# shanglianlm0525/CvPytorch

Hardware: AMD Instinct MI355X
Metric: images/sec/node train step, YOLOv5-s@640 (value: batch resident in HBM when the timed region starts; with_h2d.value: the same step fed from pinned host memory inside the region) & DeepLabv3+R50@1024x512 (config3_deeplabv3plus_r50.value) (higher is better)
Workload: dtype bf16; 1 GPU; coco_yolov5_s.yml YOLOv5-s 640x640 bf16 train step (fwd+loss+bwd+SGD-nesterov+EMA), per-GPU batch 64, synthetic COCO-shape tensors resident in HBM; global_batch=64, parallelism=dp1, launch=hipGraph replay of the whole step, world=1, transport=none (single process), grad_buckets=0, sync_bn=False, deterministic=True

## Files before the change

### cvpytorch_amd/csrc/api.hip

```cpp
#include <string.h>

#include <string>

#include "common.h"
#include "conv_plan.h"

namespace cvhip {

static thread_local std::string g_last_error = "";

void set_last_error(const char* what, hipError_t e) {
  g_last_error = std::string(what) + ": " + hipGetErrorString(e);
}

int check_launch(const char* what) {
  hipError_t e = hipGetLastError();
  if (e != hipSuccess) {
    set_last_error(what, e);
    return CVHIP_ERR_LAUNCH;
  }
  return CVHIP_OK;
}

__global__ __launch_bounds__(256) void zero_fill_kernel(uint32_t* p, size_t n_words, int tail_half) {
// ... 433 lines not shown
  p.res_ld = addend_ld;
  p.y_vec_ok = ((d->x_ld & 3) == 0) && ((((uintptr_t)dx) & 7) == 0);
  return launch_igemm(p, (hipStream_t)stream);
}

int cvhip_conv2d_dgrad(const cvhip_conv_desc* d, const void* dy, const void* w_dgrad, void* dx, void* stream) {
  return dgrad_impl(d, dy, w_dgrad, nullptr, 0, dx, stream);
}

int cvhip_conv2d_dgrad_add(const cvhip_conv_desc* d, const void* dy, const void* w_dgrad, const void* addend, int32_t addend_ld, void* dx,
                           void* stream) {
  if (!addend) return CVHIP_ERR_INVALID;
  return dgrad_impl(d, dy, w_dgrad, addend, addend_ld, dx, stream);
}

int cvhip_conv2d_wgrad(const cvhip_conv_desc* d, const void* x, const void* dy, float* dw, int accumulate, void* stream) {
  int st = validate_dense_desc(d);
  if (st) return st;
  if (!x || !dy || !dw) return CVHIP_ERR_INVALID;
  if ((d->K & 7) || (d->y_ld & 7)) return CVHIP_ERR_UNSUPPORTED;
  if ((((uintptr_t)x) & 15) || (((uintptr_t)dy) & 15)) return CVHIP_ERR_INVALID;
  hipStream_t s = (hipStream_t)stream;
  if (!accumulate) {
    int zs = zero_fill(dw, sizeof(float) * (size_t)d->K * d->R * d->S * d->C, s);
    if (zs) return zs;
  }
  return launch_wgrad(d, x, dy, dw, s);
}

int64_t cvhip_conv2d_wgrad_det_workspace_bytes(const cvhip_conv_desc* d) {
// ... 37 lines not shown
```

### cvpytorch_amd/csrc/conv1x1_stream.hip

```cpp
#include <stdlib.h>

#include "common.h"
#include "conv_plan.h"

namespace cvhip {

constexpr int kS1MaxLds = 72 * 1024;
constexpr int kS1MaxBlocks = 512;
constexpr int kS1MinTiles = 192;


template <int NV>
__device__ __forceinline__ void s1_act_vec(float (&v)[NV], int act, float ap) {
  switch (act) {
    case CVHIP_ACT_NONE: break;
    case CVHIP_ACT_RELU:
#pragma unroll
      for (int q = 0; q < NV; ++q) v[q] = act_fwd(v[q], CVHIP_ACT_RELU, ap);
      break;
    case CVHIP_ACT_SILU:
#pragma unroll
      for (int q = 0; q < NV; ++q) v[q] = act_fwd(v[q], CVHIP_ACT_SILU, ap);
      break;
    case CVHIP_ACT_LEAKY:
// ... 267 lines not shown
          u1 += red[(w * BN + t) * 2 + 0];
          u2 += red[(w * BN + t) * 2 + 1];
        }
        if (p.stats_acc) {
          acc_add2(reinterpret_cast<double*>(p.stats), blockIdx.x, p.stats_ld, n0 + t, u1, u2);
        } else {
          float* dst = p.stats + (int64_t)blockIdx.x * 2 * p.Nout;
          dst[n0 + t] = u1;
          dst[p.Nout + n0 + t] = u2;
        }
      }
    }
  }
}


static int s1x1_mode() {
  static int v = -1;
  if (v < 0) {
    const char* e = getenv("CVHIP_S1X1");
    v = e ? atoi(e) : 1;
  }
  return v;
}

static int s1x1_nf(int Nout, int Cin, bool stats) {
  if (Nout <= 32) return 2;
  if (Nout <= 64) return 4;
  if (Nout > 128 && Nout <= 256 && !stats && 256 * (((Cin + 31) & ~31) * 2 + 16) <= kS1MaxLds) return 16;
  return 8;
// ... 17 lines not shown

static bool s1x1_structural(const IgemmParams& p) {
  if (p.ncls != 1) return false;
  const IgemmClass& c = p.cls[0];
  return c.TR == 1 && c.TS == 1 && p.in_sh == 1 && p.in_sw == 1 && p.out_sh == 1 && p.out_sw == 1 && c.dh0 == 0 && c.dw0 == 0 &&
         c.out_oh == 0 && c.out_ow == 0 && c.OHi == p.OH && c.OWi == p.OW && p.IH == p.OH && p.IW == p.OW && (p.x_ld & 7) == 0;
}

static int s1x1_lds(int bn, int cin_pad, bool pro) {
  int lds = bn * (cin_pad * 2 + 16) + 5 * bn * (int)sizeof(float) + (pro ? 2 * cin_pad * (int)sizeof(float) : 0);
  if (lds < 4 * bn * 2 * (int)sizeof(float)) lds = 4 * bn * 2 * (int)sizeof(float);
  return lds;
}
constexpr int kS1MaxLdsPro = kS1MaxLds + 4096;

template <int NF, int STATS, bool EPI = false, bool PRO = false>
static int launch_s1(const IgemmParams& p, int blocks, int ntiles, hipStream_t stream) {
  constexpr int MF = 2;
  const int bn = NF * 16;
  const int cin_pad = (p.Cin + 31) & ~31;
  const int lds = s1x1_lds(bn, cin_pad, PRO);
  if (lds > kS1MaxLdsPro) return CVHIP_ERR_UNSUPPORTED;
  auto kern = conv1x1_stream_kernel<NF, MF, STATS, EPI, PRO>;
  static bool attr_done[64] = {};
  int devid = 0;
  (void)hipGetDevice(&devid);
  bool& attr_set = attr_done[devid & 63];
  if (!attr_set) {
    hipError_t e = hipFuncSetAttribute(reinterpret_cast<const void*>(kern), hipFuncAttributeMaxDynamicSharedMemorySize, kS1MaxLds + 4096);
    if (e != hipSuccess) {
      set_last_error("hipFuncSetAttribute(conv1x1_stream_kernel)", e);
      return CVHIP_ERR_LAUNCH;
    }
    attr_set = true;
  }
  const int vec16 = ((p.y_ld & 7) == 0) && ((((uintptr_t)p.y) & 15) == 0);
  const IgemmKernArgs k = narrow_plan(p, 0, 1);
  hipLaunchKernelGGL(kern, dim3(blocks, cdiv(p.Nout, bn)), dim3(256), lds, stream, k, ntiles, vec16);
  return check_launch("conv1x1_stream_kernel");
}

bool stream1x1_prologue_ok(const IgemmParams& p, bool stats) {
  if (!s1x1_structural(p)) return false;
  if (stream1x1_blocks(p.Nout, p.Cin, p.cls[0].M, stats) <= 0) return false;
  const int nf = s1x1_nf(p.Nout, p.Cin, stats);
  if (nf == 16) return false;
  return s1x1_lds(nf * 16, (p.Cin + 31) & ~31, true) <= kS1MaxLdsPro;
}

int try_launch_stream1x1(const IgemmParams& p, hipStream_t stream) {
  if (!s1x1_structural(p)) return -1;
  const int64_t M = p.cls[0].M;
  const int blocks = stream1x1_blocks(p.Nout, p.Cin, M, p.stats != nullptr);
  if (blocks <= 0) return -1;
// ... 38 lines not shown
```

### cvpytorch_amd/csrc/conv_plan.h

```cpp
#pragma once
#include <hip/hip_runtime.h>
#include <stdint.h>

#include "common.h"

namespace cvhip {

constexpr int kMaxClasses = 16;

struct IgemmClass {
  int TR, TS;
  int dh0, dh_step;
  int dw0, dw_step;
  int out_oh, out_ow;
  int OHi, OWi;
  int M;
  int tile_begin;
  int64_t w_off;
  unsigned ts_magic;
  unsigned ohw_mul, ohw_sh, ow_mul, ow_sh;
  int r0, r_step, s0, s_step;
};

struct IgemmCommon {
// ... 129 lines not shown
    return 0;
  }
  *r0 = first;
  *d0 = (ph + pad - first * dil) / stride;
  return (R - 1 - first) / step + 1;
}

int validate_dense_desc(const cvhip_conv_desc* d);
void plan_fprop(const cvhip_conv_desc* d, IgemmParams* p);
int plan_dgrad(const cvhip_conv_desc* d, IgemmParams* p);
int igemm_block_m(int Nout, int64_t M, int Ktot);
int launch_igemm(IgemmParams& p, hipStream_t stream);
int stream1x1_blocks(int Nout, int Cin, int64_t M, bool stats);
int try_launch_stream1x1(const IgemmParams& p, hipStream_t stream);
bool stream1x1_prologue_ok(const IgemmParams& p, bool stats);
int stem_blocks(int C, int x_ld, int K, int R, int S, int sh, int sw, int dh, int dw, int N, int OH, int OW);
int try_launch_stem(const IgemmParams& p, hipStream_t stream);
struct StemWgradBn {
  const void* y;
  int y_ld;
  const float *scale, *shift, *mean, *invstd;
  const double* acc;
  int acc_ld;
  int act;
  float act_param;
  float *dgamma_out, *dbeta_out;
  int accumulate;
};
int try_launch_stem_wgrad(const cvhip_conv_desc* d, const void* x, const void* dy, float* dw, hipStream_t stream, const float* x_image = nullptr,
                          int x_planes = 0, const StemWgradBn* bn = nullptr);
// ... 8 lines not shown
```

### cvpytorch_amd/csrc/f16_names.h

```cpp
#pragma once
#define cvhip_adamw_ema cvhip_adamw_ema_f16
#define cvhip_add2d cvhip_add2d_f16
#define cvhip_add_act_fwd cvhip_add_act_fwd_f16
#define cvhip_bn_acc_shards cvhip_bn_acc_shards_f16
#define cvhip_bn_act_bwd_apply cvhip_bn_act_bwd_apply_f16
#define cvhip_bn_act_bwd_apply_acc cvhip_bn_act_bwd_apply_acc_f16
#define cvhip_bn_act_bwd_partial cvhip_bn_act_bwd_partial_f16
#define cvhip_bn_act_bwd_sums_acc cvhip_bn_act_bwd_sums_acc_f16
#define cvhip_bn_act_fwd cvhip_bn_act_fwd_f16
#define cvhip_bn_act_fwd_acc cvhip_bn_act_fwd_acc_f16
#define cvhip_bn_act_fwd_acc_lazyres cvhip_bn_act_fwd_acc_lazyres_f16
#define cvhip_bn_add_act_fwd cvhip_bn_add_act_fwd_f16
#define cvhip_bn_bwd_finalize cvhip_bn_bwd_finalize_f16
#define cvhip_bn_eval_scale_shift cvhip_bn_eval_scale_shift_f16
#define cvhip_bn_finalize cvhip_bn_finalize_f16
#define cvhip_bn_finalize_acc cvhip_bn_finalize_acc_f16
#define cvhip_bn_stats_partial cvhip_bn_stats_partial_f16
#define cvhip_bn_tail_bwd_sums_acc cvhip_bn_tail_bwd_sums_acc_f16
#define cvhip_box_iou cvhip_box_iou_f16
#define cvhip_channel_scale_bwd_ds cvhip_channel_scale_bwd_ds_f16
#define cvhip_colreduce_rows cvhip_colreduce_rows_f16
#define cvhip_colsum_finalize cvhip_colsum_finalize_f16
#define cvhip_colsum_partial cvhip_colsum_partial_f16
#define cvhip_conv1x1_bwd_fused cvhip_conv1x1_bwd_fused_f16
#define cvhip_conv1x1_bwd_fused_acc cvhip_conv1x1_bwd_fused_acc_f16
#define cvhip_conv1x1_bwd_fused_lazy cvhip_conv1x1_bwd_fused_lazy_f16
#define cvhip_conv1x1_bwd_fused_ok cvhip_conv1x1_bwd_fused_ok_f16
#define cvhip_conv1x1_bwd_fused_split cvhip_conv1x1_bwd_fused_split_f16
#define cvhip_conv1x1_stream_blocks cvhip_conv1x1_stream_blocks_f16
#define cvhip_conv1x1_stream_prologue_ok cvhip_conv1x1_stream_prologue_ok_f16
#define cvhip_conv2d_band_plan cvhip_conv2d_band_plan_f16
#define cvhip_conv2d_dgrad cvhip_conv2d_dgrad_f16
#define cvhip_conv2d_dgrad_add cvhip_conv2d_dgrad_add_f16
#define cvhip_conv2d_dgrad_plan cvhip_conv2d_dgrad_plan_f16
#define cvhip_conv2d_dgrad_weight_elems cvhip_conv2d_dgrad_weight_elems_f16
#define cvhip_conv2d_fprop cvhip_conv2d_fprop_f16
#define cvhip_conv2d_fprop_acc cvhip_conv2d_fprop_acc_f16
#define cvhip_conv2d_fprop_fused cvhip_conv2d_fprop_fused_f16
#define cvhip_conv2d_fprop_prologue_ok cvhip_conv2d_fprop_prologue_ok_f16
#define cvhip_conv2d_fprop_stats_rows cvhip_conv2d_fprop_stats_rows_f16
#define cvhip_conv2d_out_hw cvhip_conv2d_out_hw_f16
#define cvhip_conv2d_patch_plan cvhip_conv2d_patch_plan_f16
#define cvhip_conv2d_prep_weights cvhip_conv2d_prep_weights_f16
// ... 78 lines not shown
```

### cvpytorch_amd/lib.py

```python
import ctypes as C
import os

import torch

_HERE = os.path.dirname(os.path.abspath(__file__))
LIB_PATH = os.environ.get("CVHIP_LIB") or os.path.join(_HERE, "libcvhip.so")

OK, ERR_INVALID, ERR_UNSUPPORTED, ERR_LAUNCH = 0, -1, -2, -3
ACT_NONE, ACT_RELU, ACT_SILU, ACT_LEAKY, ACT_SIGMOID, ACT_HSWISH = 0, 1, 2, 3, 4, 5
DTYPE_F32, DTYPE_F64, DTYPE_I32, DTYPE_BF16, DTYPE_U8 = 0, 1, 2, 3, 4
RED_SUM, RED_MAX, RED_MIN = 0, 1, 2
DGRAD_CLASS_INTS = 12
REDUCE_SCRATCH_ROWS = 64
YOLO_BIAS_ROWS = 256
BN_ACC_SHARDS = 16


class CvhipError(RuntimeError):
    pass


class ConvDesc(C.Structure):
    _fields_ = [(n, C.c_int32) for n in (
        "N", "C", "H", "W", "K", "R", "S", "stride_h", "stride_w", "pad_h", "pad_w", "dil_h", "dil_w",
# ... 60 lines not shown
    "cvhip_conv2d_dgrad_plan": (_i32, [_dp, C.POINTER(_i32), _i32]),
    "cvhip_div31_consts": (_i32, [_i32, C.POINTER(C.c_uint32), C.POINTER(C.c_uint32)]),
    "cvhip_conv2d_prep_weights": (_i32, [_dp, _p, _p, _p, _p]),
    "cvhip_prep_plan_item_bytes": (_i32, []),
    "cvhip_prep_plan_build": (_i32, [_p, _i32, _p, C.POINTER(_i32)]),
    "cvhip_prep_plan_run": (_i32, [_p, _i32, _i32, _p]),
    "cvhip_conv2d_fprop": (_i32, [_dp, _p, _p, _p, _p, _p, _p]),
    "cvhip_conv2d_fprop_fused": (_i32, [_dp, _p, _p, _p, C.POINTER(ConvFuse), _p]),
    "cvhip_conv2d_wgrad_image": (_i32, [_dp, _p, _i32, _p, _p, _p]),
    "cvhip_conv2d_fprop_prologue_ok": (_i32, [_dp, _i32]),
    "cvhip_conv2d_patch_plan": (_i32, [_dp, _i32, C.POINTER(_i32), _i32]),
    "cvhip_conv2d_band_plan": (_i32, [_dp, _i32, C.POINTER(_i32)]),
    "cvhip_conv2d_wgrad_band_plan": (_i32, [_dp, C.POINTER(_i32)]),
    "cvhip_conv1x1_stream_prologue_ok": (_i32, [_dp, _i32]),
    "cvhip_conv2d_wgrad_stem_bn": (_i32, [_dp, _p, _p, _i32, _p, _p, _p, _p, _p, _p, _p, _i32, _p, _p, _i32, _i32, _f32, _p, _p]),
    "cvhip_bn_finalize_acc": (_i32, [_p, _i32, _i32, _i64, _p, _p, _p, _p, _f32, _f32, _p, _p, _p, _p, _p]),
    "cvhip_bn_act_fwd_acc_lazyres": (_i32, [_p, _i32, _p, _i32, _i64, _i32, _p, _i32, _i64, _p, _p, _p, _p, _f32, _f32, _p, _p, _p, _p, _i32, _f32,
                                     _p, _i32, _p, _p, _p]),
    "cvhip_conv1x1_bwd_fused_split": (_i32, [_dp, _p, _i32, _p, _i32, _i32, _p, _p, _i32, _p, _p, _p, _p, _p, _p, _p, _i32, _p, _p, _i32, _i32, _f32, _p,
                                      _i32, _p, _i32, _p, C.POINTER(LazyIn), _p]),
    "cvhip_conv1x1_bwd_fused_lazy": (_i32, [_dp, _p, _i32, _p, _i32, _i32, _p, _p, _p, _p, _p, _p, _p, _p, _i32, _p, _p, _i32, _i32, _f32, _p, _i32,
                                     _p, _i32, _p, C.POINTER(LazyIn), _p]),
    "cvhip_conv2d_dgrad": (_i32, [_dp, _p, _p, _p, _p]),
    "cvhip_conv2d_dgrad_add": (_i32, [_dp, _p, _p, _p, _i32, _p, _p]),
    "cvhip_conv2d_wgrad": (_i32, [_dp, _p, _p, _p, _i32, _p]),
    "cvhip_conv2d_wgrad_det_workspace_bytes": (_i64, [_dp]),
    "cvhip_conv2d_wgrad_det": (_i32, [_dp, _p, _p, _p, _i32, _p, _i64, _p]),
    "cvhip_conv1x1_bwd_fused_ok": (_i32, [_dp]),
    "cvhip_conv1x1_bwd_fused": (_i32, [_dp, _p, _i32, _p, _i32, _i32, _p, _p, _p, _p, _p, _p, _p, _p, _p, _i32, _f32, _p, _i32, _p, _i32,
                                _p, _p]),
# ... 211 lines not shown
```

### cvpytorch_amd/ops.py

```python
import ctypes as C

import torch

from . import lib as L

ACT_DTYPE = torch.bfloat16
_weights_epoch = 0
_stats_epoch = [0]


def set_precision(p):
    global ACT_DTYPE
    L.set_precision(p)
    ACT_DTYPE = torch.float16 if p == "fp16" else torch.bfloat16
    bump_weights_epoch()
    _desc_cache.clear()


def precision():
    return L.PRECISION


def bump_weights_epoch():
    global _weights_epoch
# ... 684 lines not shown
                    g_out.data_ptr(), b_out.data_ptr(), int(accum), act, act_param, tmp.data_ptr(), st,
                    nbytes=2.0 * (N * H * W * Cc + 2 * N * P * Q * K))
    except L.CvhipError as e:
        if "unsupported" not in str(e):
            raise
        return False
    arena = cfg.arena
    direct_w = arena is not None and cfg.gw is not None and tuple(cfg.gw.shape) == tuple(weight.shape)
    if direct_w:
        L.call("cvhip_f32_unpad_add", tmp.data_ptr(), cfg.gw.data_ptr(), K, R * S, Cc, Cg, st)
        _mark(arena, cfg.idx_w)
        return None
    dw = zero_fill(torch.empty((K, Cg, R, S), dtype=torch.float32, device=dev, memory_format=torch.channels_last))
    L.call("cvhip_f32_unpad_add", tmp.data_ptr(), dw.data_ptr(), K, R * S, Cc, Cg, st)
    return dw if dw.dtype == weight.dtype else dw.to(weight.dtype)


def _bwd1x1_ok(ctx, cfg, x, need_dx, need_dw, need_db, segs):
    N, Cc, H, W, K, R, S, P, Q, Kp, x_ld, Cg = ctx.geom
    if _DETERMINISTIC:
        return False
    if ctx.depthwise or R != 1 or S != 1 or Kp != K or Cg != Cc or ctx.c_orig != Cc or not (need_dx and need_dw):
        return False
    if (ctx.has_bias and need_db) or ctx.w_dgrad is None or x.data_ptr() % 16 or x_ld % 8:
        return False
    for d, d_ld in segs:
        if d_ld % 8 or d.data_ptr() % 16:
            return False
    desc = conv_desc(N, Cc, H, W, K, R, S, cfg.stride, cfg.pad, cfg.dil, 1, x_ld, Kp)
    return bool(L.load().cvhip_conv1x1_bwd_fused_ok(C.byref(desc)))
# ... 480 lines not shown
                    need_dg = need_dbeta = False
                    for i in cfg.idx_bn:
                        arena.mark_ready(i)
                ag, ab = (dgamma, dbeta) if cfg.sync is None else _sync_bwd_sums(dgamma, dbeta, cfg.sync)
            dx, dw = _bwd1x1(ctx, cfg, x, y, weight, ((dz, dz_ld),), K, stats, ctx.train_bn, ag, ab, act, act_param)
            dres = dz if ctx.has_res else None
            if dres is not None and cfg.res_link is not None and cfg.res_link.ok:
                cfg.res_link.g = dres
                dres = None
            return dx, dw, None, (dgamma if need_dg else None), (dbeta if need_dbeta else None), None, None, dres, None
        if pointwise:
            if Kp != K:
                dy = zero_fill(torch.empty((N, P, Q, Kp), dtype=ACT_DTYPE, device=dev)).permute(0, 3, 1, 2)[:, :K]
            else:
                dy = empty_nhwc(N, K, P, Q, dev)
            if acc_b is not None:
                _timed_ew("bn_act_bwd_apply(ew_kernel<1>)", 6.0 * M * K, "cvhip_bn_act_bwd_apply_acc", dz.data_ptr(), dz_ld, y.data_ptr(), Kp, dy.data_ptr(), Kp, M, K,
                          stats[2].data_ptr(), stats[3].data_ptr(), stats[0].data_ptr(), stats[1].data_ptr(), acc_b.data_ptr(), K,
                          g_out.data_ptr(), b_out.data_ptr(), accum, act, act_param, st)
                if direct_bn:
                    need_dg = need_dbeta = False
                    for i in cfg.idx_bn:
                        arena.mark_ready(i)
            elif ctx.train_bn:
                rows = _colreduce_rows(M, K)
                partial = torch.empty((rows + L.REDUCE_SCRATCH_ROWS, 2, K), dtype=torch.float32, device=dev)
                _timed_ew("bn_act_bwd_sums(colreduce_kernel<1>)", 4.0 * M * K, "cvhip_bn_act_bwd_partial", dz.data_ptr(), dz_ld, y.data_ptr(), Kp, M, K, stats[2].data_ptr(),
                       stats[3].data_ptr(), stats[0].data_ptr(), stats[1].data_ptr(), act, act_param,
                       partial.data_ptr(), st)
                dgamma = torch.empty((K,), dtype=torch.float32, device=dev)
                dbeta = torch.empty((K,), dtype=torch.float32, device=dev)
                L.call("cvhip_bn_bwd_finalize", partial.data_ptr(), rows, K, dgamma.data_ptr(), dbeta.data_ptr(),
                       cfg.gg.data_ptr() if direct_bn else None, cfg.gbeta.data_ptr() if direct_bn else None, st)
                if direct_bn:
                    need_dg = need_dbeta = False
                    for i in cfg.idx_bn:
                        arena.mark_ready(i)
                ag, ab = (dgamma, dbeta) if cfg.sync is None else _sync_bwd_sums(dgamma, dbeta, cfg.sync)
                _timed_ew("bn_act_bwd_apply(ew_kernel<1>)", 6.0 * M * K, "cvhip_bn_act_bwd_apply", dz.data_ptr(), dz_ld, y.data_ptr(), Kp, dy.data_ptr(), Kp, M, K,
                          stats[2].data_ptr(), stats[3].data_ptr(), stats[0].data_ptr(), stats[1].data_ptr(),
                       ag.data_ptr(), ab.data_ptr(), act, act_param, st)
            else:
                sc = stats[2].data_ptr() if stats is not None else None
                sh = stats[3].data_ptr() if stats is not None else None
                L.call("cvhip_bn_act_bwd_apply", dz.data_ptr(), dz_ld, y.data_ptr(), Kp, dy.data_ptr(), Kp, M, K, sc, sh,
                       None, None, None, None, act, act_param, st)
            dy_ld = Kp
        else:
            dy, dy_ld = dz, dz_ld
            if dy_ld % 8 != 0 or dy.data_ptr() % 16 != 0 or (Kp != K and dy_ld < Kp):
                buf = zero_fill(torch.empty((N, P, Q, Kp), dtype=ACT_DTYPE, device=dev))
                L.call("cvhip_copy2d", dy.data_ptr(), dy_ld, buf.data_ptr(), Kp, M, K, st)
                dy, dy_ld = buf.permute(0, 3, 1, 2)[:, :K], Kp
        dx, dw, dbias = _conv_grads(ctx, x, weight, dy, dy_ld, need_dx, need_dw, need_db)
        dres = dz if ctx.has_res else None
        if dres is not None and cfg.res_link is not None and cfg.res_link.ok:
            cfg.res_link.g = dres
            dres = None
        if dx is not None and ctx.c_orig != Cc:
            dx = dx[:, :ctx.c_orig]
        return dx, dw, dbias, (dgamma if need_dg else None), (dbeta if need_dbeta else None), None, None, dres, None


def _lazy_consumer_ok(x, K, R, S, has_bias, cfg, lz):
    if not _LAZY or _DETERMINISTIC or not torch.is_grad_enabled() or not x.requires_grad:
        return False
    if cfg.groups != 1 or (R, S) != (1, 1) or tuple(cfg.stride) != (1, 1) or tuple(cfg.pad) != (0, 0) or has_bias:
        return False
    if not (cfg.has_bn and cfg.bn_training) or cfg.sync is not None or not _BN_ACC or K > 128 or K % 8:
# ... 1192 lines not shown
```

### include/cvhip.h

```cpp
#if !defined(CVHIP_H_) || defined(CVHIP_REDECLARE_F16)
#ifndef CVHIP_H_
#define CVHIP_H_
#endif

#include <stddef.h>
#include <stdint.h>

#ifdef __cplusplus
extern "C" {
#endif

#define CVHIP_VERSION 100

#define CVHIP_OK 0
#define CVHIP_ERR_INVALID (-1)
#define CVHIP_ERR_UNSUPPORTED (-2)
#define CVHIP_ERR_LAUNCH (-3)

#define CVHIP_ACT_NONE 0
#define CVHIP_ACT_RELU 1
#define CVHIP_ACT_SILU 2
#define CVHIP_ACT_LEAKY 3
#define CVHIP_ACT_SIGMOID 4
#define CVHIP_ACT_HSWISH 5
// ... 377 lines not shown
  const float* scale;
  const float* shift;
  int32_t act;
  float act_param;
  int32_t c_lo;
  int32_t c_hi;
} cvhip_lazy_in;
#endif
int cvhip_conv2d_fprop_fused(const cvhip_conv_desc* d, const void* x, const void* w, void* y, const cvhip_conv_fuse* f, void* stream);
int cvhip_conv2d_wgrad_image(const cvhip_conv_desc* d, const float* x_nchw, int32_t planes, const void* dy, float* dw, void* stream);
int cvhip_conv2d_wgrad_stem_bn(const cvhip_conv_desc* d, const void* x, const float* x_nchw, int32_t planes, const void* dz, const void* y,
                               const float* scale, const float* shift, const float* mean, const float* invstd, const double* acc, int32_t acc_ld,
                               float* dgamma_out, float* dbeta_out, int32_t accumulate, int32_t act, float act_param, float* dw, void* stream);
int cvhip_conv2d_fprop_prologue_ok(const cvhip_conv_desc* d, int with_z_out);
int cvhip_conv1x1_stream_prologue_ok(const cvhip_conv_desc* d, int with_stats);
int cvhip_bn_finalize_acc(const double* acc, int32_t acc_ld, int32_t C, int64_t count, const float* gamma, const float* beta,
                          float* running_mean, float* running_var, float momentum, float eps, float* mean, float* invstd, float* scale,
                          float* shift, void* stream);
int cvhip_bn_act_fwd_acc_lazyres(const void* y, int32_t ld_y, void* z, int32_t ld_z, int64_t M, int32_t C, const double* acc, int32_t acc_ld,
                                 int64_t count, const float* gamma, const float* beta, float* running_mean, float* running_var,
                                 float momentum, float eps, float* mean, float* invstd, float* scale, float* shift, int32_t act,
                                 float act_param, const void* residual_raw, int32_t ld_res, const float* res_scale, const float* res_shift,
                                 void* stream);
int cvhip_conv1x1_bwd_fused_split(const cvhip_conv_desc* d, const void* dz0, int32_t dz0_ld, const void* dz1, int32_t dz1_ld, int32_t k_split,
                                  const void* y, const void* y1, int32_t y1_ld, const void* x, const void* w_dgrad, const float* scale,
                                  const float* shift, const float* mean, const float* invstd, const double* acc, int32_t acc_ld,
                                  float* dgamma_out, float* dbeta_out, int32_t accumulate, int32_t act, float act_param, const void* addend,
                                  int32_t addend_ld, void* dx, int32_t dx_ld, float* dw, const cvhip_lazy_in* xin, void* stream);
int cvhip_conv1x1_bwd_fused_lazy(const cvhip_conv_desc* d, const void* dz0, int32_t dz0_ld, const void* dz1, int32_t dz1_ld, int32_t k_split,
                                 const void* y, const void* x_raw, const void* w_dgrad, const float* scale, const float* shift, const float* mean,
// ... 18 lines not shown
```

### include/cvhip_f16.h

```cpp
#ifndef CVHIP_F16_H_
#define CVHIP_F16_H_
#include "cvhip.h"
#define cvhip_adamw_ema cvhip_adamw_ema_f16
#define cvhip_add2d cvhip_add2d_f16
#define cvhip_add_act_fwd cvhip_add_act_fwd_f16
#define cvhip_bn_acc_shards cvhip_bn_acc_shards_f16
#define cvhip_bn_act_bwd_apply cvhip_bn_act_bwd_apply_f16
#define cvhip_bn_act_bwd_apply_acc cvhip_bn_act_bwd_apply_acc_f16
#define cvhip_bn_act_bwd_partial cvhip_bn_act_bwd_partial_f16
#define cvhip_bn_act_bwd_sums_acc cvhip_bn_act_bwd_sums_acc_f16
#define cvhip_bn_act_fwd cvhip_bn_act_fwd_f16
#define cvhip_bn_act_fwd_acc cvhip_bn_act_fwd_acc_f16
#define cvhip_bn_act_fwd_acc_lazyres cvhip_bn_act_fwd_acc_lazyres_f16
#define cvhip_bn_add_act_fwd cvhip_bn_add_act_fwd_f16
#define cvhip_bn_bwd_finalize cvhip_bn_bwd_finalize_f16
#define cvhip_bn_eval_scale_shift cvhip_bn_eval_scale_shift_f16
#define cvhip_bn_finalize cvhip_bn_finalize_f16
#define cvhip_bn_finalize_acc cvhip_bn_finalize_acc_f16
#define cvhip_bn_stats_partial cvhip_bn_stats_partial_f16
#define cvhip_bn_tail_bwd_sums_acc cvhip_bn_tail_bwd_sums_acc_f16
#define cvhip_box_iou cvhip_box_iou_f16
#define cvhip_channel_scale_bwd_ds cvhip_channel_scale_bwd_ds_f16
#define cvhip_colreduce_rows cvhip_colreduce_rows_f16
#define cvhip_colsum_finalize cvhip_colsum_finalize_f16
#define cvhip_colsum_partial cvhip_colsum_partial_f16
#define cvhip_conv1x1_bwd_fused cvhip_conv1x1_bwd_fused_f16
#define cvhip_conv1x1_bwd_fused_acc cvhip_conv1x1_bwd_fused_acc_f16
#define cvhip_conv1x1_bwd_fused_lazy cvhip_conv1x1_bwd_fused_lazy_f16
#define cvhip_conv1x1_bwd_fused_ok cvhip_conv1x1_bwd_fused_ok_f16
#define cvhip_conv1x1_bwd_fused_split cvhip_conv1x1_bwd_fused_split_f16
#define cvhip_conv1x1_stream_blocks cvhip_conv1x1_stream_blocks_f16
#define cvhip_conv1x1_stream_prologue_ok cvhip_conv1x1_stream_prologue_ok_f16
#define cvhip_conv2d_band_plan cvhip_conv2d_band_plan_f16
#define cvhip_conv2d_dgrad cvhip_conv2d_dgrad_f16
#define cvhip_conv2d_dgrad_add cvhip_conv2d_dgrad_add_f16
#define cvhip_conv2d_dgrad_plan cvhip_conv2d_dgrad_plan_f16
#define cvhip_conv2d_dgrad_weight_elems cvhip_conv2d_dgrad_weight_elems_f16
#define cvhip_conv2d_fprop cvhip_conv2d_fprop_f16
#define cvhip_conv2d_fprop_acc cvhip_conv2d_fprop_acc_f16
#define cvhip_conv2d_fprop_fused cvhip_conv2d_fprop_fused_f16
#define cvhip_conv2d_fprop_prologue_ok cvhip_conv2d_fprop_prologue_ok_f16
#define cvhip_conv2d_fprop_stats_rows cvhip_conv2d_fprop_stats_rows_f16
#define cvhip_conv2d_out_hw cvhip_conv2d_out_hw_f16
#define cvhip_conv2d_patch_plan cvhip_conv2d_patch_plan_f16
#define cvhip_conv2d_prep_weights cvhip_conv2d_prep_weights_f16
// ... 93 lines not shown
#undef cvhip_bn_eval_scale_shift
#undef cvhip_bn_finalize
#undef cvhip_bn_finalize_acc
#undef cvhip_bn_stats_partial
#undef cvhip_bn_tail_bwd_sums_acc
#undef cvhip_box_iou
#undef cvhip_channel_scale_bwd_ds
#undef cvhip_colreduce_rows
#undef cvhip_colsum_finalize
#undef cvhip_colsum_partial
#undef cvhip_conv1x1_bwd_fused
#undef cvhip_conv1x1_bwd_fused_acc
#undef cvhip_conv1x1_bwd_fused_lazy
#undef cvhip_conv1x1_bwd_fused_ok
#undef cvhip_conv1x1_bwd_fused_split
#undef cvhip_conv1x1_stream_blocks
#undef cvhip_conv1x1_stream_prologue_ok
#undef cvhip_conv2d_band_plan
#undef cvhip_conv2d_dgrad
#undef cvhip_conv2d_dgrad_add
#undef cvhip_conv2d_dgrad_plan
#undef cvhip_conv2d_dgrad_weight_elems
#undef cvhip_conv2d_fprop
#undef cvhip_conv2d_fprop_acc
#undef cvhip_conv2d_fprop_fused
#undef cvhip_conv2d_fprop_prologue_ok
#undef cvhip_conv2d_fprop_stats_rows
#undef cvhip_conv2d_out_hw
#undef cvhip_conv2d_patch_plan
#undef cvhip_conv2d_prep_weights
// ... 79 lines not shown
```

Before: 5015 images/sec.

## Fuse BN-activation backward apply into the 1x1 conv dgrad stream kernel

Adds a variant of the streaming 1x1 conv kernel that loads dz and y, applies the BN+activation backward transform in registers, writes du (from the first N-block only), and feeds the result straight into the MFMA dgrad GEMM. The Python backward uses it instead of the separate elementwise bn_act_bwd_apply kernel whenever the geometry qualifies. dx then comes from the fused kernel and the regular dgrad is skipped. This saves one kernel launch and the re-read of du by dgrad. The cost is that each N-block recomputes the transform and loads y alongside dz, which adds register pressure and redundant work when Nout spans several blocks.

```diff
diff --git a/cvpytorch_amd/csrc/api.hip b/cvpytorch_amd/csrc/api.hip
--- a/cvpytorch_amd/csrc/api.hip
+++ b/cvpytorch_amd/csrc/api.hip
@@ -471,6 +471,62 @@
   return dgrad_impl(d, dy, w_dgrad, addend, addend_ld, dx, stream);
 }
 
+static bool dgb_unpadded(const cvhip_conv_desc* d) { return (d->k_valid <= 0 || d->k_valid == d->K) && (d->c_valid <= 0 || d->c_valid == d->C); }
+
+int cvhip_conv1x1_dgrad_bnact_ok(const cvhip_conv_desc* d) {
+  if (validate_dense_desc(d) || (d->K & 7) || (d->y_ld & 7) || !dgb_unpadded(d)) return 0;
+  IgemmParams p;
+  plan_dgrad(d, &p);
+  return stream1x1_dgrad_bnact_ok(p) ? 1 : 0;
+}
+
+int cvhip_conv1x1_dgrad_bnact(const cvhip_conv_desc* d, const void* dz, int32_t dz_ld, const void* y, const void* w_dgrad, const float* scale,
+                              const float* shift, const float* mean, const float* invstd, const double* acc, int32_t acc_ld, float* dgamma,
+                              float* dbeta, int32_t accumulate, int32_t act, float act_param, const void* addend, int32_t addend_ld, void* du,
+                              int32_t du_ld, void* dx, void* stream) {
+  int st = validate_dense_desc(d);
+  if (st) return st;
+  if (!dz || !y || !w_dgrad || !du || !dx || !scale || !shift || !mean || !invstd) return CVHIP_ERR_INVALID;
+  if (acc ? (acc_ld < d->K || (((uintptr_t)acc) & 7)) : (!dgamma || !dbeta)) return CVHIP_ERR_INVALID;
+  if ((d->K & 7) || (d->y_ld & 7) || (dz_ld & 7) || (du_ld & 7) || !dgb_unpadded(d)) return CVHIP_ERR_UNSUPPORTED;
+  if (dz_ld < d->K || du_ld < d->K || (addend && addend_ld < d->C)) return CVHIP_ERR_INVALID;
+  if ((((uintptr_t)dz) & 15) || (((uintptr_t)y) & 15) || (((uintptr_t)du) & 15) || (((uintptr_t)w_dgrad) & 15)) return CVHIP_ERR_INVALID;
+  cvhip_conv_desc dd = *d;
+  dd.y_ld = dz_ld;
+  IgemmParams p;
+  plan_dgrad(&dd, &p);
+  p.x = (const h16_t*)dz;
+  p.w = (const h16_t*)w_dgrad;
+  p.y = (h16_t*)dx;
+  p.bias = nullptr;
+  p.stats = nullptr;
+  p.stats_acc = 0;
+  p.stats_ld = d->C;
+  p.res = (const h16_t*)addend;
+  p.res_ld = addend_ld;
+  p.y_vec_ok = ((d->x_ld & 3) == 0) && ((((uintptr_t)dx) & 7) == 0);
+  S1BwdArgs bw{};
+  bw.y = (const h16_t*)y;
+  bw.y_ld = d->y_ld;
+  bw.du = (h16_t*)du;
+  bw.du_ld = du_ld;
+  bw.scale = scale;
+  bw.shift = shift;
+  bw.mean = mean;
+  bw.invstd = invstd;
+  bw.acc = acc;
+  bw.acc_ld = acc_ld;
+  bw.dgamma = acc ? nullptr : dgamma;
+  bw.dbeta = acc ? nullptr : dbeta;
+  bw.dgamma_out = acc ? dgamma : nullptr;
+  bw.dbeta_out = acc ? dbeta : nullptr;
+  bw.accumulate = accumulate;
+  bw.ap = act_param;
+  const int64_t M = (int64_t)p.cls[0].M;
+  bw.inv_count = 1.f / (float)M;
+  return launch_stream1x1_dgrad_bnact(p, bw, act, (hipStream_t)stream);
+}
+
 int cvhip_conv2d_wgrad(const cvhip_conv_desc* d, const void* x, const void* dy, float* dw, int accumulate, void* stream) {
   int st = validate_dense_desc(d);
   if (st) return st;
diff --git a/cvpytorch_amd/csrc/conv1x1_stream.hip b/cvpytorch_amd/csrc/conv1x1_stream.hip
--- a/cvpytorch_amd/csrc/conv1x1_stream.hip
+++ b/cvpytorch_amd/csrc/conv1x1_stream.hip
@@ -305,6 +305,230 @@
   }
 }
 
+template <int ACT>
+struct S1Bwd {
+  static constexpr int act = ACT;
+};
+template <int NF, int MF, typename TAG>
+__global__ __launch_bounds__(256, 2) void conv1x1_stream_kernel(const IgemmKernArgs p, int ntiles, int vec16, const S1BwdArgs bw) {
+  constexpr int BN = NF * 16;
+  constexpr int RT = 64 * MF;
+  constexpr int KC = 128 / MF;
+  constexpr int KS = KC / 32;
+  extern __shared__ __attribute__((aligned(16))) unsigned char smem[];
+
+  const int t = threadIdx.x;
+  const int lane = t & 63;
+  const int wave = __builtin_amdgcn_readfirstlane(t >> 6);
+  const int r = lane & 15, g = lane >> 4;
+  const int Cin = p.Cin;
+  const int M = p.cls[0].M;
+  const int cin_pad = (Cin + 31) & ~31;
+  const int brow = cin_pad * 2 + 16;
+  const int nkc = (cin_pad + KC - 1) / KC;
+  const int n0 = blockIdx.y * BN;
+  const int my_tiles = (ntiles - (int)blockIdx.x + (int)gridDim.x - 1) / (int)gridDim.x;
+  const int total = my_tiles * nkc;
+
+  h16x8 buf0[MF][KS], buf1[MF][KS], ybuf0[MF][KS], ybuf1[MF][KS];
+
+  int ld_tile = blockIdx.x, ld_kc = 0;
+  auto load = [&](h16x8 (&dst)[MF][KS], h16x8 (&ydst)[MF][KS]) {
+    const int row0 = ld_tile * RT + wave * (MF * 16) + r;
+    const int kbase = ld_kc * KC + g * 8;
+#pragma unroll
+    for (int b = 0; b < MF; ++b) {
+      int m = row0 + b * 16;
+      m = m < M ? m : M - 1;
+      const h16_t* src = p.x + (int64_t)m * p.x_ld;
+      const h16_t* ysrc = bw.y + (int64_t)m * bw.y_ld;
+#pragma unroll
+      for (int ks = 0; ks < KS; ++ks) {
+        int kk = kbase + ks * 32;
+        kk = kk < Cin ? kk : 0;
+        dst[b][ks] = *reinterpret_cast<const h16x8*>(src + kk);
+        ydst[b][ks] = *reinterpret_cast<const h16x8*>(ysrc + kk);
+      }
+    }
+    if (++ld_kc == nkc) {
+      ld_kc = 0;
+      ld_tile += gridDim.x;
+    }
+  };
+  load(buf0, ybuf0);
+
+  {
+    const int cpr = cin_pad >> 3;
+    const int nchunks = BN * cpr;
+    constexpr int U = 8;
+    for (int q0 = t; q0 < nchunks; q0 += 256 * U) {
+      uint4 v[U];
+      int dst[U];
+#pragma unroll
+      for (int u = 0; u < U; ++u) {
+        const int q = q0 + u * 256;
+        const int L = q / cpr;
+        const int kq = q - L * cpr;
+        const int a = L >> 4, i = L & 15;
+        const int ch = n0 + (a >> 1) * 32 + (i >> 2) * 8 + (a & 1) * 4 + (i & 3);
+        dst[u] = q < nchunks ? L * brow + kq * 16 : -1;
+        v[u] = make_uint4(0u, 0u, 0u, 0u);
+        if (q < nchunks && ch < p.Nout && kq * 8 < Cin) v[u] = *reinterpret_cast<const uint4*>(p.w + (int64_t)ch * Cin + kq * 8);
+      }
+#pragma unroll
+      for (int u = 0; u < U; ++u)
+        if (dst[u] >= 0) *reinterpret_cast<uint4*>(smem + dst[u]) = v[u];
+    }
+  }
+  float* const scst = reinterpret_cast<float*>(smem + BN * brow);
+  for (int c = t; c < cin_pad; c += 256) {
+    const int cc = c < Cin ? c : Cin - 1;
+    float k1, k2;
+    if (bw.acc) {
+      double s1, s2;
+      acc_fold2(bw.acc, bw.acc_ld, cc, s1, s2);
+      k1 = (float)s1 * bw.inv_count;
+      k2 = (float)s2 * bw.inv_count;
+      if (blockIdx.x == 0 && blockIdx.y == 0 && c < Cin) {
+        if (bw.dbeta_out) bw.dbeta_out[c] = bw.accumulate ? bw.dbeta_out[c] + (float)s1 : (float)s1;
+        if (bw.dgamma_out) bw.dgamma_out[c] = bw.accumulate ? bw.dgamma_out[c] + (float)s2 : (float)s2;
+      }
+    } else {
+      k1 = bw.dbeta[cc] * bw.inv_count;
+      k2 = bw.dgamma[cc] * bw.inv_count;
+    }
+    scst[c] = bw.scale[cc];
+    scst[cin_pad + c] = bw.shift[cc];
+    scst[2 * cin_pad + c] = bw.mean[cc];
+    scst[3 * cin_pad + c] = bw.invstd[cc];
+    scst[4 * cin_pad + c] = k1;
+    scst[5 * cin_pad + c] = k2;
+  }
+  __syncthreads();
+
+  f32x4 acc[NF][MF];
+#pragma unroll
+  for (int a = 0; a < NF; ++a)
+#pragma unroll
+    for (int b = 0; b < MF; ++b) acc[a][b] = f32x4{0.f, 0.f, 0.f, 0.f};
+
+  const unsigned char* const wlane = smem + r * brow + g * 16;
+  int cp_tile = blockIdx.x, cp_kc = 0;
+
+  auto xform = [&](h16x8 (&buf)[MF][KS], const h16x8 (&ybuf)[MF][KS]) {
+    const int kbase = cp_kc * KC + g * 8;
+    const int ksn = min(KS, (cin_pad - cp_kc * KC) >> 5);
+    const int row0 = cp_tile * RT + wave * (MF * 16) + r;
+    const bool keep = blockIdx.y == 0;
+#pragma unroll
+    for (int ks = 0; ks < KS; ++ks) {
+      const int kk = kbase + ks * 32;
+      if (ks < ksn && kk < Cin) {
+        uint32_t dw[MF][4], yw[MF][4];
+#pragma unroll
+        for (int b = 0; b < MF; ++b) {
+          const uint4 d4 = __builtin_bit_cast(uint4, buf[b][ks]), y4 = __builtin_bit_cast(uint4, ybuf[b][ks]);
+          dw[b][0] = d4.x; dw[b][1] = d4.y; dw[b][2] = d4.z; dw[b][3] = d4.w;
+          yw[b][0] = y4.x; yw[b][1] = y4.y; yw[b][2] = y4.z; yw[b][3] = y4.w;
+        }
+#pragma unroll
+        for (int h = 0; h < 2; ++h) {
+          const float* cs = scst + kk + 4 * h;
+          const f32x4 sc = *reinterpret_cast<const f32x4*>(cs), sh = *reinterpret_cast<const f32x4*>(cs + cin_pad);
+          const f32x4 mu = *reinterpret_cast<const f32x4*>(cs + 2 * cin_pad), is = *reinterpret_cast<const f32x4*>(cs + 3 * cin_pad);
+          const f32x4 k1 = *reinterpret_cast<const f32x4*>(cs + 4 * cin_pad), k2 = *reinterpret_cast<const f32x4*>(cs + 5 * cin_pad);
+#pragma unroll
+          for (int b = 0; b < MF; ++b)
+#pragma unroll
+            for (int q = 0; q < 2; ++q) {
+              const int e = 2 * q, w = 2 * h + q;
+              const f32x2 o = bnact_bwd_apply2<TAG::act, true>(unpack_pair(dw[b][w]), unpack_pair(yw[b][w]), f32x2{sc[e], sc[e + 1]},
+                                                               f32x2{sh[e], sh[e + 1]}, f32x2{mu[e], mu[e + 1]}, f32x2{is[e], is[e + 1]},
+                                                               f32x2{k1[e], k1[e + 1]}, f32x2{k2[e], k2[e + 1]}, bw.ap);
+              dw[b][w] = pack2(o.x, o.y);
+            }
+        }
+#pragma unroll
+        for (int b = 0; b < MF; ++b) {
+          const uint4 o4 = make_uint4(dw[b][0], dw[b][1], dw[b][2], dw[b][3]);
+          buf[b][ks] = __builtin_bit_cast(h16x8, o4);
+          const int m = row0 + b * 16;
+          if (keep && m < M) *reinterpret_cast<uint4*>(bw.du + (int64_t)m * bw.du_ld + kk) = o4;
+        }
+      }
+    }
+  };
+
+  auto compute = [&](const h16x8 (&src)[MF][KS]) {
+    const unsigned char* wk = wlane + cp_kc * (KC * 2);
+    const int ksn = min(KS, (cin_pad - cp_kc * KC) >> 5);
+#pragma unroll
+    for (int ks = 0; ks < KS; ++ks) {
+      if (ks < ksn) {
+#pragma unroll
+        for (int a = 0; a < NF; ++a) {
+          const h16x8 wb = *reinterpret_cast<const h16x8*>(wk + a * 16 * brow + ks * 64);
+#pragma unroll
+          for (int b = 0; b < MF; ++b) acc[a][b] = CVHIP_MFMA_16X16X32(wb, src[b][ks], acc[a][b], 0, 0, 0);
+        }
+      }
+    }
+    if (++cp_kc < nkc) return;
+    const int row0 = cp_tile * RT + wave * (MF * 16) + r;
+#pragma unroll
+    for (int b = 0; b < MF; ++b) {
+      const int m = row0 + b * 16;
+      h16_t* yrow = p.y + (int64_t)m * p.y_ld;
+#pragma unroll
+      for (int j = 0; j < NF / 2; ++j) {
+        const int ch0 = n0 + j * 32 + g * 8;
+        f32x8 v;
+#pragma unroll
+        for (int q = 0; q < 4; ++q) {
+          v.v[q] = acc[2 * j][b][q];
+          v.v[4 + q] = acc[2 * j + 1][b][q];
+        }
+        if (p.res && m < M) {
+          const h16_t* rrow = p.res + (int64_t)m * p.res_ld + ch0;
+          if (ch0 + 7 < p.Nout && (p.res_ld & 7) == 0 && ((((uintptr_t)p.res) & 15) == 0)) {
+            const f32x8 rv = unpack8(*reinterpret_cast<const uint4*>(rrow));
+#pragma unroll
+            for (int q = 0; q < 8; ++q) v.v[q] += rv.v[q];
+          } else {
+#pragma unroll
+            for (int q = 0; q < 8; ++q)
+              if (ch0 + q < p.Nout) v.v[q] += (float)rrow[q];
+          }
+        }
+        if (m < M) {
+          if (vec16 && ch0 + 7 < p.Nout) {
+            *reinterpret_cast<uint4*>(yrow + ch0) = pack8(v);
+          } else {
+#pragma unroll
+            for (int q = 0; q < 8; ++q)
+              if (ch0 + q < p.Nout) yrow[ch0 + q] = (h16_t)v.v[q];
+          }
+        }
+      }
+    }
+#pragma unroll
+    for (int a = 0; a < NF; ++a)
+#pragma unroll
+      for (int b = 0; b < MF; ++b) acc[a][b] = f32x4{0.f, 0.f, 0.f, 0.f};
+    cp_kc = 0;
+    cp_tile += gridDim.x;
+  };
+
+  for (int it = 0; it < total; it += 2) {
+    load(buf1, ybuf1);
+    xform(buf0, ybuf0);
+    compute(buf0);
+    load(buf0, ybuf0);
+    xform(buf1, ybuf1);
+    compute(buf1);
+  }
+}
+
 
 static int s1x1_mode() {
   static int v = -1;
@@ -352,6 +576,21 @@
 }
 constexpr int kS1MaxLdsPro = kS1MaxLds + 4096;
 
+static int s1_grant_lds(const void* kern, bool (&done)[64]) {
+  int devid = 0;
+  (void)hipGetDevice(&devid);
+  bool& attr_set = done[devid & 63];
+  if (!attr_set) {
+    hipError_t e = hipFuncSetAttribute(kern, hipFuncAttributeMaxDynamicSharedMemorySize, kS1MaxLdsPro);
+    if (e != hipSuccess) {
+      set_last_error("hipFuncSetAttribute(conv1x1_stream_kernel)", e);
+      return CVHIP_ERR_LAUNCH;
+    }
+    attr_set = true;
+  }
+  return CVHIP_OK;
+}
+
 template <int NF, int STATS, bool EPI = false, bool PRO = false>
 static int launch_s1(const IgemmParams& p, int blocks, int ntiles, hipStream_t stream) {
   constexpr int MF = 2;
@@ -361,21 +600,68 @@
   if (lds > kS1MaxLdsPro) return CVHIP_ERR_UNSUPPORTED;
   auto kern = conv1x1_stream_kernel<NF, MF, STATS, EPI, PRO>;
   static bool attr_done[64] = {};
-  int devid = 0;
-  (void)hipGetDevice(&devid);
-  bool& attr_set = attr_done[devid & 63];
-  if (!attr_set) {
-    hipError_t e = hipFuncSetAttribute(reinterpret_cast<const void*>(kern), hipFuncAttributeMaxDynamicSharedMemorySize, kS1MaxLds + 4096);
-    if (e != hipSuccess) {
-      set_last_error("hipFuncSetAttribute(conv1x1_stream_kernel)", e);
-      return CVHIP_ERR_LAUNCH;
-    }
-    attr_set = true;
-  }
+  if (const int st = s1_grant_lds(reinterpret_cast<const void*>(kern), attr_done)) return st;
   const int vec16 = ((p.y_ld & 7) == 0) && ((((uintptr_t)p.y) & 15) == 0);
   const IgemmKernArgs k = narrow_plan(p, 0, 1);
   hipLaunchKernelGGL(kern, dim3(blocks, cdiv(p.Nout, bn)), dim3(256), lds, stream, k, ntiles, vec16);
   return check_launch("conv1x1_stream_kernel");
+}
+
+static int s1x1_dgb_nf(int Nout, int Cin) {
+  const int nf = s1x1_nf(Nout, Cin, false);
+  return nf == 16 ? 8 : nf;
+}
+static int s1x1_dgb_lds(int bn, int cin_pad) { return bn * (cin_pad * 2 + 16) + 6 * cin_pad * (int)sizeof(float); }
+
+static int s1x1_dgb_blocks(const IgemmParams& p) {
+  if (!s1x1_structural(p) || (p.Cin & 7)) return 0;
+  const int64_t M = p.cls[0].M;
+  const int blocks = stream1x1_blocks(p.Nout, p.Cin, M, false);
+  if (blocks <= 0) return 0;
+  const int bn = s1x1_dgb_nf(p.Nout, p.Cin) * 16;
+  if (s1x1_mode() == 1 && p.Nout > bn && (double)M * p.Cin * 2.0 > 64e6) return 0;
+  if (s1x1_dgb_lds(bn, (p.Cin + 31) & ~31) > kS1MaxLds) return 0;
+  return blocks;
+}
+
+bool stream1x1_dgrad_bnact_ok(const IgemmParams& p) {
+  if (s1x1_dgb_blocks(p) <= 0) return false;
+  return s1x1_mode() != 1 || p.Nout <= s1x1_dgb_nf(p.Nout, p.Cin) * 16;
+}
+
+template <int NF, int ACT>
+static int launch_s1_dgb(const IgemmParams& p, const S1BwdArgs& bw, int blocks, int ntiles, hipStream_t stream) {
+  const int bn = NF * 16;
+  auto kern = conv1x1_stream_kernel<NF, 2, S1Bwd<ACT>>;
+  static bool attr_done[64] = {};
+  if (const int st = s1_grant_lds(reinterpret_cast<const void*>(kern), attr_done)) return st;
+  const int vec16 = ((p.y_ld & 7) == 0) && ((((uintptr_t)p.y) & 15) == 0);
+  const IgemmKernArgs k = narrow_plan(p, 0, 1);
+  hipLaunchKernelGGL(kern, dim3(blocks, cdiv(p.Nout, bn)), dim3(256), s1x1_dgb_lds(bn, (p.Cin + 31) & ~31), stream, k, ntiles, vec16, bw);
+  return check_launch("conv1x1_stream_kernel<dgrad_bnact>");
+}
+
+template <int NF>
+static int launch_s1_dgb_act(const IgemmParams& p, const S1BwdArgs& bw, int act, int blocks, int ntiles, hipStream_t stream) {
+  switch (act) {
+    case CVHIP_ACT_NONE: return launch_s1_dgb<NF, CVHIP_ACT_NONE>(p, bw, blocks, ntiles, stream);
+    case CVHIP_ACT_RELU: return launch_s1_dgb<NF, CVHIP_ACT_RELU>(p, bw, blocks, ntiles, stream);
+    case CVHIP_ACT_SILU: return launch_s1_dgb<NF, CVHIP_ACT_SILU>(p, bw, blocks, ntiles, stream);
+    case CVHIP_ACT_LEAKY: return launch_s1_dgb<NF, CVHIP_ACT_LEAKY>(p, bw, blocks, ntiles, stream);
+    case CVHIP_ACT_SIGMOID: return launch_s1_dgb<NF, CVHIP_ACT_SIGMOID>(p, bw, blocks, ntiles, stream);
+    case CVHIP_ACT_HSWISH: return launch_s1_dgb<NF, CVHIP_ACT_HSWISH>(p, bw, blocks, ntiles, stream);
+    default: return CVHIP_ERR_INVALID;
+  }
+}
+
+int launch_stream1x1_dgrad_bnact(const IgemmParams& p, const S1BwdArgs& bw, int act, hipStream_t stream) {
+  const int blocks = s1x1_dgb_blocks(p);
+  if (blocks <= 0) return CVHIP_ERR_UNSUPPORTED;
+  const int ntiles = (int)(((int64_t)p.cls[0].M + 127) / 128);
+  const int nf = s1x1_dgb_nf(p.Nout, p.Cin);
+  if (nf == 2) return launch_s1_dgb_act<2>(p, bw, act, blocks, ntiles, stream);
+  if (nf == 4) return launch_s1_dgb_act<4>(p, bw, act, blocks, ntiles, stream);
+  return launch_s1_dgb_act<8>(p, bw, act, blocks, ntiles, stream);
 }
 
 bool stream1x1_prologue_ok(const IgemmParams& p, bool stats) {
diff --git a/cvpytorch_amd/csrc/conv_plan.h b/cvpytorch_amd/csrc/conv_plan.h
--- a/cvpytorch_amd/csrc/conv_plan.h
+++ b/cvpytorch_amd/csrc/conv_plan.h
@@ -167,6 +167,19 @@
 int stream1x1_blocks(int Nout, int Cin, int64_t M, bool stats);
 int try_launch_stream1x1(const IgemmParams& p, hipStream_t stream);
 bool stream1x1_prologue_ok(const IgemmParams& p, bool stats);
+struct S1BwdArgs {
+  const h16_t* y;
+  h16_t* du;
+  int y_ld, du_ld;
+  const float *scale, *shift, *mean, *invstd;
+  const double* acc;
+  const float *dgamma, *dbeta;
+  float *dgamma_out, *dbeta_out;
+  int acc_ld, accumulate;
+  float ap, inv_count;
+};
+bool stream1x1_dgrad_bnact_ok(const IgemmParams& p);
+int launch_stream1x1_dgrad_bnact(const IgemmParams& p, const S1BwdArgs& bw, int act, hipStream_t stream);
 int stem_blocks(int C, int x_ld, int K, int R, int S, int sh, int sw, int dh, int dw, int N, int OH, int OW);
 int try_launch_stem(const IgemmParams& p, hipStream_t stream);
 struct StemWgradBn {
diff --git a/cvpytorch_amd/csrc/f16_names.h b/cvpytorch_amd/csrc/f16_names.h
--- a/cvpytorch_amd/csrc/f16_names.h
+++ b/cvpytorch_amd/csrc/f16_names.h
@@ -27,6 +27,8 @@
 #define cvhip_conv1x1_bwd_fused_lazy cvhip_conv1x1_bwd_fused_lazy_f16
 #define cvhip_conv1x1_bwd_fused_ok cvhip_conv1x1_bwd_fused_ok_f16
 #define cvhip_conv1x1_bwd_fused_split cvhip_conv1x1_bwd_fused_split_f16
+#define cvhip_conv1x1_dgrad_bnact cvhip_conv1x1_dgrad_bnact_f16
+#define cvhip_conv1x1_dgrad_bnact_ok cvhip_conv1x1_dgrad_bnact_ok_f16
 #define cvhip_conv1x1_stream_blocks cvhip_conv1x1_stream_blocks_f16
 #define cvhip_conv1x1_stream_prologue_ok cvhip_conv1x1_stream_prologue_ok_f16
 #define cvhip_conv2d_band_plan cvhip_conv2d_band_plan_f16
diff --git a/cvpytorch_amd/lib.py b/cvpytorch_amd/lib.py
--- a/cvpytorch_amd/lib.py
+++ b/cvpytorch_amd/lib.py
@@ -98,6 +98,8 @@
     "cvhip_conv2d_wgrad_band_plan": (_i32, [_dp, C.POINTER(_i32)]),
     "cvhip_conv1x1_stream_prologue_ok": (_i32, [_dp, _i32]),
     "cvhip_conv2d_wgrad_stem_bn": (_i32, [_dp, _p, _p, _i32, _p, _p, _p, _p, _p, _p, _p, _i32, _p, _p, _i32, _i32, _f32, _p, _p]),
+    "cvhip_conv1x1_dgrad_bnact": (_i32, [_dp, _p, _i32, _p, _p, _p, _p, _p, _p, _p, _i32, _p, _p, _i32, _i32, _f32, _p, _i32, _p, _i32, _p, _p]),
+    "cvhip_conv1x1_dgrad_bnact_ok": (_i32, [_dp]),
     "cvhip_bn_finalize_acc": (_i32, [_p, _i32, _i32, _i64, _p, _p, _p, _p, _f32, _f32, _p, _p, _p, _p, _p]),
     "cvhip_bn_act_fwd_acc_lazyres": (_i32, [_p, _i32, _p, _i32, _i64, _i32, _p, _i32, _i64, _p, _p, _p, _p, _f32, _f32, _p, _p, _p, _p, _i32, _f32,
                                      _p, _i32, _p, _p, _p]),
diff --git a/cvpytorch_amd/ops.py b/cvpytorch_amd/ops.py
--- a/cvpytorch_amd/ops.py
+++ b/cvpytorch_amd/ops.py
@@ -722,6 +722,38 @@
     dw = zero_fill(torch.empty((K, Cg, R, S), dtype=torch.float32, device=dev, memory_format=torch.channels_last))
     L.call("cvhip_f32_unpad_add", tmp.data_ptr(), dw.data_ptr(), K, R * S, Cc, Cg, st)
     return dw if dw.dtype == weight.dtype else dw.to(weight.dtype)
+
+
+def _dgrad_bnact_ok(ctx, cfg, dz, dz_ld, y, need_dx):
+    N, Cc, H, W, K, R, S, P, Q, Kp, x_ld, Cg = ctx.geom
+    if not need_dx or not ctx.train_bn or cfg.sync is not None or ctx.depthwise or ctx.w_dgrad is None:
+        return False
+    if not _pointwise(R, S, cfg) or Kp != K or Cg != Cc or K % 8 or dz_ld % 8 or dz.data_ptr() % 16 or y.data_ptr() % 16:
+        return False
+    desc = conv_desc(N, Cc, H, W, K, R, S, cfg.stride, cfg.pad, cfg.dil, 1, Cc, Kp)
+    query = getattr(L.load(), "cvhip_conv1x1_dgrad_bnact_ok", None)
+    return query is not None and bool(query(C.byref(desc)))
+
+
+def _dgrad_bnact(ctx, cfg, dz, dz_ld, y, stats, dy, act, act_param, acc, g, b, accum):
+    N, Cc, H, W, K, R, S, P, Q, Kp, x_ld, Cg = ctx.geom
+    st = _stream()
+    dx = empty_nhwc(N, Cc, H, W, dz.device)
+    desc = conv_desc(N, Cc, H, W, K, R, S, cfg.stride, cfg.pad, cfg.dil, 1, Cc, Kp)
+    a, a_ld = None, 0
+    link = cfg.dx_link
+    if link is not None and link.g is not None and ctx.c_orig == Cc:
+        a, a_ld = as_nhwc(link.g)
+        link.g = None
+        if tuple(a.shape) != (N, Cc, H, W):
+            raise L.CvhipError("GradLink: skip-connection gradient %s does not match the layer input %s" % (tuple(a.shape), (N, Cc, H, W)))
+    M = N * P * Q
+    _timed_call("conv1x1_stream_kernel<%d>+bnact_bwd" % (32 if Cc <= 32 else 64 if Cc <= 64 else 128), (N, Cc, H, W, K, R, S, P, Q),
+                "cvhip_conv1x1_dgrad_bnact", C.byref(desc), dz.data_ptr(), dz_ld, y.data_ptr(), ctx.w_dgrad.data_ptr(),
+                stats[2].data_ptr(), stats[3].data_ptr(), stats[0].data_ptr(), stats[1].data_ptr(), _ptr(acc), K, g.data_ptr(), b.data_ptr(),
+                int(accum), act, act_param, _ptr(a), a_ld, dy.data_ptr(), Kp, dx.data_ptr(), st,
+                nbytes=2.0 * (3 * M * K + M * Cc * (2 if a is not None else 1) + K * Cc))
+    return dx
 
 
 def _bwd1x1_ok(ctx, cfg, x, need_dx, need_dw, need_db, segs):
@@ -1232,10 +1264,15 @@
                 dy = zero_fill(torch.empty((N, P, Q, Kp), dtype=ACT_DTYPE, device=dev)).permute(0, 3, 1, 2)[:, :K]
             else:
                 dy = empty_nhwc(N, K, P, Q, dev)
+            dx_fused = None
+            on_load = _dgrad_bnact_ok(ctx, cfg, dz, dz_ld, y, need_dx)
             if acc_b is not None:
-                _timed_ew("bn_act_bwd_apply(ew_kernel<1>)", 6.0 * M * K, "cvhip_bn_act_bwd_apply_acc", dz.data_ptr(), dz_ld, y.data_ptr(), Kp, dy.data_ptr(), Kp, M, K,
-                          stats[2].data_ptr(), stats[3].data_ptr(), stats[0].data_ptr(), stats[1].data_ptr(), acc_b.data_ptr(), K,
-                          g_out.data_ptr(), b_out.data_ptr(), accum, act, act_param, st)
+                if on_load:
+                    dx_fused = _dgrad_bnact(ctx, cfg, dz, dz_ld, y, stats, dy, act, act_param, acc_b, g_out, b_out, accum)
+                else:
+                    _timed_ew("bn_act_bwd_apply(ew_kernel<1>)", 6.0 * M * K, "cvhip_bn_act_bwd_apply_acc", dz.data_ptr(), dz_ld, y.data_ptr(), Kp, dy.data_ptr(), Kp, M, K,
+                              stats[2].data_ptr(), stats[3].data_ptr(), stats[0].data_ptr(), stats[1].data_ptr(), acc_b.data_ptr(), K,
+                              g_out.data_ptr(), b_out.data_ptr(), accum, act, act_param, st)
                 if direct_bn:
                     need_dg = need_dbeta = False
                     for i in cfg.idx_bn:
@@ -1255,9 +1292,12 @@
                     for i in cfg.idx_bn:
                         arena.mark_ready(i)
                 ag, ab = (dgamma, dbeta) if cfg.sync is None else _sync_bwd_sums(dgamma, dbeta, cfg.sync)
-                _timed_ew("bn_act_bwd_apply(ew_kernel<1>)", 6.0 * M * K, "cvhip_bn_act_bwd_apply", dz.data_ptr(), dz_ld, y.data_ptr(), Kp, dy.data_ptr(), Kp, M, K,
-                          stats[2].data_ptr(), stats[3].data_ptr(), stats[0].data_ptr(), stats[1].data_ptr(),
-                       ag.data_ptr(), ab.data_ptr(), act, act_param, st)
+                if on_load:
+                    dx_fused = _dgrad_bnact(ctx, cfg, dz, dz_ld, y, stats, dy, act, act_param, None, ag, ab, 0)
+                else:
+                    _timed_ew("bn_act_bwd_apply(ew_kernel<1>)", 6.0 * M * K, "cvhip_bn_act_bwd_apply", dz.data_ptr(), dz_ld, y.data_ptr(), Kp, dy.data_ptr(), Kp, M, K,
+                              stats[2].data_ptr(), stats[3].data_ptr(), stats[0].data_ptr(), stats[1].data_ptr(),
+                              ag.data_ptr(), ab.data_ptr(), act, act_param, st)
             else:
                 sc = stats[2].data_ptr() if stats is not None else None
                 sh = stats[3].data_ptr() if stats is not None else None
@@ -1265,12 +1305,15 @@
                        None, None, None, None, act, act_param, st)
             dy_ld = Kp
         else:
+            dx_fused = None
             dy, dy_ld = dz, dz_ld
             if dy_ld % 8 != 0 or dy.data_ptr() % 16 != 0 or (Kp != K and dy_ld < Kp):
                 buf = zero_fill(torch.empty((N, P, Q, Kp), dtype=ACT_DTYPE, device=dev))
                 L.call("cvhip_copy2d", dy.data_ptr(), dy_ld, buf.data_ptr(), Kp, M, K, st)
                 dy, dy_ld = buf.permute(0, 3, 1, 2)[:, :K], Kp
-        dx, dw, dbias = _conv_grads(ctx, x, weight, dy, dy_ld, need_dx, need_dw, need_db)
+        dx, dw, dbias = _conv_grads(ctx, x, weight, dy, dy_ld, need_dx and dx_fused is None, need_dw, need_db)
+        if dx_fused is not None:
+            dx = dx_fused
         dres = dz if ctx.has_res else None
         if dres is not None and cfg.res_link is not None and cfg.res_link.ok:
             cfg.res_link.g = dres
diff --git a/include/cvhip.h b/include/cvhip.h
--- a/include/cvhip.h
+++ b/include/cvhip.h
@@ -415,6 +415,11 @@
                                float* dgamma_out, float* dbeta_out, int32_t accumulate, int32_t act, float act_param, float* dw, void* stream);
 int cvhip_conv2d_fprop_prologue_ok(const cvhip_conv_desc* d, int with_z_out);
 int cvhip_conv1x1_stream_prologue_ok(const cvhip_conv_desc* d, int with_stats);
+int cvhip_conv1x1_dgrad_bnact(const cvhip_conv_desc* d, const void* dz, int32_t dz_ld, const void* y, const void* w_dgrad, const float* scale,
+                              const float* shift, const float* mean, const float* invstd, const double* acc, int32_t acc_ld, float* dgamma,
+                              float* dbeta, int32_t accumulate, int32_t act, float act_param, const void* addend, int32_t addend_ld, void* du,
+                              int32_t du_ld, void* dx, void* stream);
+int cvhip_conv1x1_dgrad_bnact_ok(const cvhip_conv_desc* d);
 int cvhip_bn_finalize_acc(const double* acc, int32_t acc_ld, int32_t C, int64_t count, const float* gamma, const float* beta,
                           float* running_mean, float* running_var, float momentum, float eps, float* mean, float* invstd, float* scale,
                           float* shift, void* stream);
diff --git a/include/cvhip_f16.h b/include/cvhip_f16.h
--- a/include/cvhip_f16.h
+++ b/include/cvhip_f16.h
@@ -29,6 +29,8 @@
 #define cvhip_conv1x1_bwd_fused_lazy cvhip_conv1x1_bwd_fused_lazy_f16
 #define cvhip_conv1x1_bwd_fused_ok cvhip_conv1x1_bwd_fused_ok_f16
 #define cvhip_conv1x1_bwd_fused_split cvhip_conv1x1_bwd_fused_split_f16
+#define cvhip_conv1x1_dgrad_bnact cvhip_conv1x1_dgrad_bnact_f16
+#define cvhip_conv1x1_dgrad_bnact_ok cvhip_conv1x1_dgrad_bnact_ok_f16
 #define cvhip_conv1x1_stream_blocks cvhip_conv1x1_stream_blocks_f16
 #define cvhip_conv1x1_stream_prologue_ok cvhip_conv1x1_stream_prologue_ok_f16
 #define cvhip_conv2d_band_plan cvhip_conv2d_band_plan_f16
@@ -152,6 +154,8 @@
 #undef cvhip_conv1x1_bwd_fused_lazy
 #undef cvhip_conv1x1_bwd_fused_ok
 #undef cvhip_conv1x1_bwd_fused_split
+#undef cvhip_conv1x1_dgrad_bnact
+#undef cvhip_conv1x1_dgrad_bnact_ok
 #undef cvhip_conv1x1_stream_blocks
 #undef cvhip_conv1x1_stream_prologue_ok
 #undef cvhip_conv2d_band_plan
```

After: 5031 images/sec (median of 6 runs). No clear change (+0.3%).
